# chalharu/rust-compression

Hardware: AMD Instinct MI355X
Metric: BZip2 level-9 encode MB/s (input bytes, HBM-resident in and out: the kernels' rate; value_end_to_end is host buffer to host buffer at the C ABI) (higher is better)
Workload: dtype u8/u32

## Files before the change

rust-compression_amd/csrc/bzgpu.h:

```cpp
#pragma once
#include <hip/hip_runtime.h>
#include <stdint.h>
#include <stddef.h>

namespace bzgpu {

typedef uint8_t u8;
typedef uint16_t u16;
typedef uint32_t u32;
typedef uint64_t u64;
typedef int64_t i64;

constexpr u32 kWave = 64;
constexpr u32 kMaxBlockLen = 900000;
constexpr u32 kSortTile = 8192;
constexpr u32 kSortThreads = 512;
constexpr u32 kTilesPerBlock = 110;
constexpr u32 kSlot = kTilesPerBlock * kSortTile;
constexpr u32 kMaxBins = 2048;
constexpr u32 kPerK = 8;
constexpr u32 kGSize = 50;
constexpr u32 kMaxSelectors = 18002;
constexpr u32 kMaxAlpha = 258;
constexpr u32 kRleTile = 4096;
// ... 248 lines not shown
    u32 *bin_base;
    u32 *count;
    u32 *count2;
    u32 *tile_nf;
    u8 *flags;
    u64 *newbits;
    int *tile_last_old;
    int *tile_last_new;
    u32 *nonfinal;
    unsigned long long *active;
    u32 *maxnf;
    u32 *per_k, *per_shift;
    u32 *lin_p, *lin_sig;
    u32 *bin_cursor;
    u32 *pb_gate;
    u32 *loc_stats;
    u8 *L;
    u32 *orig_ptr;
    u8 *ptext;
    const u8 *sym_code;
    const u8 *keyinfo;
    u32 *gh_tiles;
    u32 *gbase;
    u32 *tile_state;
    u32 *tickets;
    u32 *sort_err;
    u32 *epoch;
    u8 *per_aux;
    u32 per_keyshift;
    u32 per_wide;
    u32 per_links;
    u32 *fused_state;
    u32 *tile_state_all;
    u32 fused;
    size_t tile_state_bytes;
};
constexpr u32 kSortEpochs = 1024;

constexpr u32 kMtfStride = kSlot + 64;
struct MtfArgs {
    const BlockDesc *blocks;
    u32 nb;
    u32 tiles;
    const u8 *L;
    const u32 *inuse_bits;
    u8 *summ;
    u16 *summ_len;
    u8 *init_state;
    u8 *rank8;
    int *ztile_last;
    u32 *ztile_cnt;
    u32 *zstate;
    u32 *ztick;
    u32 fused_zle;
    u16 *mtf;
    u32 *mtf_freq;
    BlockOut *out;
};

constexpr u32 kLim = 17;
constexpr u32 kLmRow = 2 * kMaxAlpha + 4;
constexpr u32 kLmWords = 2 * kLim * kLmRow + 5 * kMaxAlpha + 64;
constexpr u32 kSelStride = kMaxSelectors + 14;
constexpr u32 kGboStride = kMaxSelectors + 2;
struct HuffArgs {
    const BlockDesc *blocks;
    u32 nb;
    const u16 *mtf;
    u32 mtf_stride;
    const u32 *mtf_freq;
    const u32 *inuse_bits;
    const u32 *crc;
    const u32 *orig_ptr;
    u8 *selector;
    u32 *code_len;
    u32 *group_bitoff;
    u32 *lm_scratch;
    u8 *glen;
    unsigned long long *pack;
    u32 *rfreq;
    u32 *hlm;
    u32 *pass_stats;
    u32 *stream;
    BlockOut *out;
    u32 *error_flag;
};

struct AsmBlock {
    u64 src_word;
    u64 bit_len;
    u64 dst_bit;
};
struct PackBlock {
    u64 src_word, dst_word, nwords;
};

constexpr int BZ_DEC_E_DATA = -1;
struct DecCand {
    u64 bitpos;
    u32 type;
    u32 pad;
};
struct DecBlockInfo {
    u64 end_bit;
    u32 status;
    u32 stored_crc;
// ... 139 lines not shown
```

rust-compression_amd/csrc/engine.hip:

```cpp
#include "engine_state.h"

#include <algorithm>
#include <chrono>
#include <cstdio>
#include <cstdlib>
#include <cstring>
#include <vector>


#define MAILCHK(st, ...)                                                             \
    do {                                                                             \
        const MailSeg mail_segs_[] = {__VA_ARGS__};                                  \
        if (mail_fetch((st), mail_segs_, (int)(sizeof(mail_segs_) / sizeof(mail_segs_[0]))) != 0) return BZ_E_UNEXPECTED; \
    } while (0)

static int span_begin(bz_gpu_engine *g, int stage, hipStream_t st = nullptr)
{
    bz_gpu_engine::Span s;
    s.stage = stage;
    s.st = st ? st : g->st;
    if (hipEventCreate(&s.a) != hipSuccess || hipEventCreate(&s.b) != hipSuccess) return -1;
    (void)hipEventRecord(s.a, s.st);
    g->spans.push_back(s);
    return (int)g->spans.size() - 1;
// ... 26 lines not shown
static int ensure_workspace(bz_gpu_engine *g, size_t need_blocks)
{
    if (need_blocks > g->max_blocks) need_blocks = g->max_blocks;
    if (need_blocks < 8) need_blocks = 8;
    if (g->ws_blocks >= need_blocks) return BZ_OK;
    size_t nb = need_blocks + need_blocks / 4;
    if (nb > g->max_blocks) nb = g->max_blocks;
    int rc = BZ_OK;
    g->ws_blocks = 0;
#define ENS(buf, bytes)                         \
    do {                                        \
        rc = g->buf.ensure((size_t)(bytes));    \
        if (rc != BZ_OK) return rc;             \
    } while (0)
    ENS(lblocks, nb * sizeof(BlockDesc));
    ENS(lcrc, nb * 4);
    ENS(SA, nb * (size_t)kSlot * 4);
    ENS(R, nb * (size_t)kSlot * 4);
    ENS(KA, nb * (size_t)kSlot * 4);
    ENS(VA, nb * (size_t)kSlot * 4);
    ENS(KB, nb * (size_t)kSlot * 4);
    ENS(VB, nb * (size_t)kSlot * 4);
    ENS(tile_hist, nb * (size_t)kTilesPerBlock * kMaxBins * 4);
    ENS(count, nb * 4);
    ENS(bin_base, nb * (size_t)kMaxBins * 4);
    ENS(sym_code, nb * (size_t)256);
    ENS(count2, nb * 4);
    ENS(tile_nf, nb * (size_t)kTilesPerBlock * 4);
    ENS(keyinfo, nb * (size_t)4);
    ENS(flags, nb * (size_t)kSlot);
    ENS(newbits, nb * (size_t)kSlot / 8 + 256);
    ENS(tlo, nb * (size_t)kTilesPerBlock * 4);
    ENS(tln, nb * (size_t)kTilesPerBlock * 4);
    ENS(nonfinal, nb * 4);
    ENS(active, 64 * 8 + 64 * 4);
    ENS(per_k, nb * 4);
    ENS(per_shift, nb * 4);
    ENS(lin_p, nb * (size_t)4 * kPerK);
    ENS(lin_sig, nb * (size_t)4 * kPerK);
    ENS(bin_cursor, nb * (size_t)1024 * 4);
    ENS(pb_gate, nb * (size_t)4 + 1024);
    if (hipMemsetAsync(g->pb_gate.p, 0, g->pb_gate.cap, g->st) != hipSuccess) return BZ_E_UNEXPECTED;
    ENS(L, nb * (size_t)kSlot + 64);
    ENS(orig_ptr, nb * 4);
    ENS(inuse_bits, nb * 32);
    ENS(summ, nb * (size_t)kMaxMtfChunks * 256);
    ENS(summ_len, nb * (size_t)kMaxMtfChunks * 2);
    ENS(init_state, nb * (size_t)kMaxMtfChunks * 256);
    ENS(rank8, nb * (size_t)kSlot + 64);
    ENS(ztile_last, nb * (size_t)kTilesPerBlock * 4);
    ENS(ztile_cnt, nb * (size_t)kTilesPerBlock * 4);
    ENS(zstate, nb * (size_t)kTilesPerBlock * 16);
    ENS(ztick, 64);
    ENS(mtf, nb * (size_t)kMtfStride * 2);
    ENS(mtf_freq, nb * (size_t)kMaxAlpha * 4);
    ENS(bout, nb * sizeof(BlockOut));
    ENS(selector, nb * (size_t)kSelStride);
    ENS(code_len, nb * (size_t)6 * kMaxAlpha * 4);
    ENS(group_bitoff, nb * (size_t)kGboStride * 4);
    ENS(lm_scratch, nb * (size_t)6 * kLmWords * 4);
    ENS(hglen, nb * (size_t)6 * (kMaxAlpha + 6));
    ENS(hpack, nb * (size_t)kMaxAlpha * 8);
    ENS(hrfreq, nb * (size_t)6 * kMaxAlpha * 4);
    ENS(hlm, nb * 4);
    ENS(hpass, nb * (size_t)32 * 4);
    ENS(stream, nb * (size_t)kStreamWords * 4);
    ENS(error_flag, 4);
    ENS(packlist, nb * sizeof(PackBlock));
    if (fused_wanted()) {
        ENS(gh_tiles, nb * (size_t)kTilesPerBlock * 3 * kMaxBins * 4);
        ENS(gbase, nb * (size_t)3 * kMaxBins * 4);
        ENS(tile_state, nb * (size_t)kTilesPerBlock * kMaxBins * 4);
        ENS(tickets, (size_t)kSortEpochs * 8 * 4 + 64);
        if (hipMemsetAsync(g->tile_state.p, 0, g->tile_state.cap, g->st) != hipSuccess ||
            hipMemsetAsync(g->tickets.p, 0, g->tickets.cap, g->st) != hipSuccess)
            return BZ_E_UNEXPECTED;
        g->sort_epoch = 0;
    }
#undef ENS
    g->ws_blocks = nb;
    return BZ_OK;
}

extern "C" int bz_device_count(void)
{
    int n = 0;
    if (hipGetDeviceCount(&n) != hipSuccess) return 0;
    return n;
}

extern "C" size_t bz_encode_bound(size_t n)
{
    return n + n / 2 + (n / 700000 + 2) * 24576 + 64;
}

extern "C" int bz_gpu_engine_create(bz_gpu_engine **out, int device, size_t max_blocks_in_flight)
{
    if (!out) return BZ_E_PARAM;
    *out = nullptr;
    int ndev = 0;
    if (hipGetDeviceCount(&ndev) != hipSuccess || ndev <= 0) return BZ_E_NOGPU;
    if (device < 0 || device >= ndev) return BZ_E_PARAM;
    HIPCHK(hipSetDevice(device));
    bz_gpu_engine *g = new bz_gpu_engine();
    g->device = device;
    g->max_blocks = max_blocks_in_flight ? max_blocks_in_flight : 64;
    g->verify = bzgpu::env_verify();
    HIPCHK(hipStreamCreateWithFlags(&g->st, hipStreamNonBlocking));
    HIPCHK(hipStreamCreateWithFlags(&g->st2, hipStreamNonBlocking));
    HIPCHK(hipHostMalloc((void **)&g->h_active, 64, hipHostMallocDefault));

    u32 tab[256], xp16[256], xp2[48];
    for (u32 i = 0; i < 256; ++i) {
        u32 v = i << 24;
        for (int k = 0; k < 8; ++k) v = (v & 0x80000000u) ? ((v << 1) ^ kCrcPoly) : (v << 1);
        tab[i] = v;
    }
    xp2[0] = 0x100u;
    for (int k = 1; k < 48; ++k) xp2[k] = gf_mulmod(xp2[k - 1], xp2[k - 1]);
    xp16[0] = 1u;
    for (int k = 1; k < 256; ++k) xp16[k] = gf_mulmod(xp16[k - 1], xp2[4]);
    int rc;
    if ((rc = g->crc_tab.ensure(sizeof(tab))) || (rc = g->xp16.ensure(sizeof(xp16))) ||
        (rc = g->xp2.ensure(sizeof(xp2)))) {
        delete g;
        return rc;
    }
    HIPCHK(hipMemcpy(g->crc_tab.p, tab, sizeof(tab), hipMemcpyHostToDevice));
    HIPCHK(hipMemcpy(g->xp16.p, xp16, sizeof(xp16), hipMemcpyHostToDevice));
    HIPCHK(hipMemcpy(g->xp2.p, xp2, sizeof(xp2), hipMemcpyHostToDevice));
    *out = g;
    return BZ_OK;
}

extern "C" int bz_gpu_engine_reserve(bz_gpu_engine *g, size_t blocks)
{
    if (!g) return BZ_E_PARAM;
    HIPCHK(hipSetDevice(g->device));
    return ensure_workspace(g, blocks);
}

extern "C" void bz_gpu_engine_destroy(bz_gpu_engine *g)
{
    if (!g) return;
    (void)hipSetDevice(g->device);
    (void)hipStreamSynchronize(g->st);
    (void)hipStreamSynchronize(g->st2);
    DevBuf *all[] = {&g->dec_in, &g->oneshot_out, &g->cut_step_t0, &g->cut_step_nt, &g->cut_step_w0, &g->cut_tab, &g->cut_comp,
                     &g->crc_tab, &g->xp16, &g->xp2, &g->tile_last, &g->carry_in, &g->tile_crc, &g->tile_count,
                     &g->tile_off, &g->sub_off, &g->sub_rs, &g->scal, &g->scan_part, &g->rle, &g->blocks_all, &g->crc_all, &g->lblocks, &g->lcrc, &g->SA,
                     &g->R, &g->KA, &g->VA, &g->KB, &g->VB, &g->tile_hist, &g->count, &g->flags, &g->tlo, &g->tln,
                     &g->nonfinal, &g->active, &g->per_k, &g->per_shift, &g->lin_p, &g->lin_sig, &g->bin_cursor, &g->pb_gate, &g->newbits, &g->bin_base, &g->sym_code, &g->keyinfo, &g->count2, &g->tile_nf, &g->L, &g->orig_ptr, &g->inuse_bits,
                     &g->summ, &g->summ_len, &g->init_state, &g->rank8, &g->ztile_last, &g->ztile_cnt, &g->mtf,
                     &g->mtf_freq, &g->bout, &g->selector, &g->code_len, &g->group_bitoff, &g->lm_scratch, &g->hglen, &g->hpack, &g->hrfreq, &g->hlm, &g->hpass,
                     &g->stream, &g->error_flag, &g->packlist, &g->packed, &g->gathered, &g->asmlist, &g->gh_tiles, &g->gbase, &g->tile_state,
                     &g->tickets, &g->vstream, &g->vout, &g->vseg, &g->vmis};
    for (DevBuf *b : all) b->release();
    dec_workspace_free(g->dec);
    df_workspace_free(g->df);
    if (g->h_active) (void)hipHostFree(g->h_active);
    if (g->st) (void)hipStreamDestroy(g->st);
    if (g->ev_aux) (void)hipEventDestroy(g->ev_aux);
    if (g->st2) (void)hipStreamDestroy(g->st2);
    delete g;
}

static RleBuffers rle_buffers(bz_gpu_engine *g)
{
    RleBuffers rb;
    rb.tile_last = g->tile_last.as<i64>();
    rb.carry_in = g->carry_in.as<i64>();
    rb.tile_crc = g->tile_crc.as<u32>();
    rb.tile_count = g->tile_count.as<u32>();
    rb.tile_off = g->tile_off.as<u64>();
    rb.sub_off = g->sub_off.as<u16>();
    rb.sub_rs = g->sub_rs.as<i64>();
    rb.total = g->scal.as<u64>();
    rb.cut_result = g->scal.as<u64>() + 2;
    rb.scan_part = g->scan_part.as<u64>();
    return rb;
}

extern "C" int bz_gpu_partition_slab_begin(bz_gpu_engine *g, int level, const void *d_in, size_t n,
                                           uint64_t tile0, uint64_t tile1, int64_t *slab_last_start)
{
    if (!g || level < 1 || level > 9) return BZ_E_PARAM;
    if (n && ((uintptr_t)d_in & 15u)) return BZ_E_PARAM;
    HIPCHK(hipSetDevice(g->device));
    const u64 ntiles = (n + kRleTile - 1) / kRleTile;
    if (tile1 > ntiles) tile1 = ntiles;
    if (tile0 > tile1) tile0 = tile1;
    g->level = level;
    g->d_in = (const u8 *)d_in;
    g->n_in = n;
    g->slab_t0 = tile0;
    g->slab_t1 = tile1;
    g->h_blocks.clear();
    g->h_crc.clear();
    for (double &t : g->t_stage) t = 0;
    for (u64 &s : g->bwt_stats) s = 0;
    for (u64 &s : g->round_active) s = 0;
    if (slab_last_start) *slab_last_start = -1;
    if (ntiles == 0) return BZ_OK;
    int rc;
    if ((rc = g->tile_last.ensure(ntiles * 8)) || (rc = g->carry_in.ensure(ntiles * 8)) ||
        (rc = g->tile_crc.ensure(ntiles * 4)) || (rc = g->tile_count.ensure(ntiles * 4)) ||
// ... 368 lines not shown
    x.tile_last_old = g->tlo.as<int>() + t;
    x.tile_last_new = g->tln.as<int>() + t;
    x.nonfinal = g->nonfinal.as<u32>() + o;
    x.active = g->active.as<unsigned long long>();
    x.maxnf = reinterpret_cast<u32 *>(g->active.as<unsigned long long>() + 64);
    x.per_k = g->per_k.as<u32>() + o;
    x.per_shift = g->per_shift.as<u32>() + o;
    x.lin_p = g->lin_p.as<u32>() + (size_t)o * kPerK;
    x.lin_sig = g->lin_sig.as<u32>() + (size_t)o * kPerK;
    x.bin_cursor = g->bin_cursor.as<u32>() + (size_t)o * 1024;
    x.pb_gate = g->pb_gate.as<u32>() + o;
    x.loc_stats = g->pb_gate.as<u32>() + g->ws_blocks;
    x.L = g->L.as<u8>() + s;
    x.orig_ptr = g->orig_ptr.as<u32>() + o;
    x.ptext = g->rank8.as<u8>() + s;
    x.sym_code = g->sym_code.as<u8>() + (size_t)o * 256;
    x.keyinfo = g->keyinfo.as<u8>() + (size_t)o * 4;
    x.gh_tiles = g->gh_tiles.as<u32>() + t * 3 * kMaxBins;
    x.gbase = g->gbase.as<u32>() + (size_t)o * 3 * kMaxBins;
    x.tile_state = g->tile_state.as<u32>() + t * kMaxBins;
    x.tickets = g->tickets.as<u32>();
    x.sort_err = g->tickets.p ? g->tickets.as<u32>() + (size_t)kSortEpochs * 8 : nullptr;
    x.epoch = &g->sort_epoch;
    x.fused_state = g->fused_state;
    x.tile_state_all = g->tile_state.as<u32>();
    x.tile_state_bytes = g->tile_state.cap;
    x.fused = fused_wanted() ? 1u : 0u;
    static const u32 want_links = (getenv("BZ_LINK_ROUND") && atoi(getenv("BZ_LINK_ROUND")) == 0) ? 0u : 1u;
    x.per_links = want_links;
    x.per_keyshift = 0;
    x.per_wide = 0;
    x.per_aux = reinterpret_cast<u8 *>(g->mtf.as<u16>() + (size_t)o * kMtfStride);
    return x;
}

static MtfArgs make_mtf_args(bz_gpu_engine *g, u32 nb, u32 o, u32 total_nb)
{
    MtfArgs ma;
    const size_t s = (size_t)o * kSlot, t = (size_t)o * kTilesPerBlock, c = (size_t)o * kMaxMtfChunks;
    ma.blocks = g->lblocks.as<BlockDesc>() + o;
    ma.nb = nb;
    ma.tiles = kTilesPerBlock;
    ma.L = g->L.as<u8>() + s;
    ma.inuse_bits = g->inuse_bits.as<u32>() + (size_t)o * 8;
    ma.summ = g->summ.as<u8>() + c * 256;
    ma.summ_len = g->summ_len.as<u16>() + c;
    ma.init_state = g->init_state.as<u8>() + c * 256;
    ma.rank8 = g->rank8.as<u8>() + s;
    ma.ztile_last = g->ztile_last.as<int>() + t;
    ma.ztile_cnt = g->ztile_cnt.as<u32>() + t;
    ma.zstate = g->zstate.as<u32>() + t * 4;
    ma.ztick = g->ztick.as<u32>();
    static const bool want_fused_zle = !(getenv("BZ_FUSED_ZLE") && atoi(getenv("BZ_FUSED_ZLE")) == 0);
    ma.fused_zle = (want_fused_zle && !g->zle_fused_broken && o == 0 && nb == total_nb) ? 1u : 0u;
    ma.mtf = g->mtf.as<u16>() + (size_t)o * kMtfStride;
    ma.mtf_freq = g->mtf_freq.as<u32>() + (size_t)o * kMaxAlpha;
    ma.out = g->bout.as<BlockOut>() + o;
    return ma;
}

static HuffArgs make_huff_args(bz_gpu_engine *g, u32 nb, u32 o)
{
    HuffArgs ha;
    ha.blocks = g->lblocks.as<BlockDesc>() + o;
    ha.nb = nb;
    ha.mtf = g->mtf.as<u16>() + (size_t)o * kMtfStride;
    ha.mtf_stride = kMtfStride;
    ha.mtf_freq = g->mtf_freq.as<u32>() + (size_t)o * kMaxAlpha;
    ha.inuse_bits = g->inuse_bits.as<u32>() + (size_t)o * 8;
    ha.crc = g->lcrc.as<u32>() + o;
    ha.orig_ptr = g->orig_ptr.as<u32>() + o;
    ha.selector = g->selector.as<u8>() + (size_t)o * kSelStride;
    ha.code_len = g->code_len.as<u32>() + (size_t)o * 6 * kMaxAlpha;
    ha.group_bitoff = g->group_bitoff.as<u32>() + (size_t)o * kGboStride;
    ha.lm_scratch = g->lm_scratch.as<u32>() + (size_t)o * 6 * kLmWords;
    ha.glen = g->hglen.as<u8>() + (size_t)o * 6 * (kMaxAlpha + 6);
    ha.pack = g->hpack.as<unsigned long long>() + (size_t)o * kMaxAlpha;
    ha.rfreq = g->hrfreq.as<u32>() + (size_t)o * 6 * kMaxAlpha;
    ha.hlm = g->hlm.as<u32>() + o;
    ha.pass_stats = g->debug_figures ? g->hpass.as<u32>() + (size_t)o * 32 : nullptr;
    ha.stream = g->stream.as<u32>() + (size_t)o * kStreamWords;
    ha.out = g->bout.as<BlockOut>() + o;
    ha.error_flag = g->error_flag.as<u32>();
    return ha;
}

__global__ void k_test_bump(u32 *p, u32 n) { *p = (*p + 1u) % n; }
__global__ void k_test_swap(u8 *L, u32 n)
{
    for (u32 i = n / 2; i + 1 < n; ++i)
        if (L[i] != L[i + 1]) {
            const u8 t = L[i];
            L[i] = L[i + 1];
            L[i + 1] = t;
            return;
        }
}

static int sort_batch(bz_gpu_engine *g, const BwtArgs &ba, u32 *inuse_bits, u32 max_n, u64 total_n, u64 *sorted,
                      KernelProf *prof, u64 *round_active)
{
    launch_block_symbols(g->st, ba, inuse_bits, const_cast<u8 *>(ba.sym_code), const_cast<u8 *>(ba.keyinfo));
    std::vector<u8> ki((size_t)ba.nb * 4);
    {
        const MailSeg sg = {ki.data(), ba.keyinfo, ki.size()};
        if (mail_fetch(g->st, &sg, 1) != 0) return -1;
    }
// ... 874 lines not shown
```

rust-compression_amd/csrc/engine_state.h:

```cpp
#pragma once
#include "../../include/bz2_mi355x.h"
#include "bzgpu.h"

#include <cstdio>
#include <vector>

using namespace bzgpu;

struct DecWorkspace;
void dec_workspace_free(DecWorkspace *w);
int dec_decode_for_verify(struct bz_gpu_engine *g, const uint8_t *d_in, uint64_t n, uint8_t *d_out, uint64_t cap,
                          uint64_t *produced, int *verdict);
struct bz_gpu_engine *dec_cache_take(int device, int prefer = 0);
void dec_cache_put(int device, struct bz_gpu_engine *g);
void dec_release_cached();
struct DfWorkspace;
void df_workspace_free(DfWorkspace *w);

#define HIPCHK(x)                                                                                     \
    do {                                                                                              \
        hipError_t e_ = (x);                                                                          \
        if (e_ != hipSuccess) {                                                                       \
            fprintf(stderr, "bz2_mi355x: HIP error %s at %s:%d\n", hipGetErrorString(e_), __FILE__,   \
                    __LINE__);                                                                        \
            return BZ_E_UNEXPECTED;                                                                   \
        }                                                                                             \
    } while (0)

struct DevBuf {
    void *p = nullptr;
    size_t cap = 0;
    int ensure(size_t bytes)
    {
        if (bytes <= cap) return BZ_OK;
        if (p) (void)hipFree(p);
        p = nullptr;
        cap = 0;
        size_t want = bytes + bytes / 8 + 256;
        if (hipMalloc(&p, want) != hipSuccess) {
            if (hipMalloc(&p, bytes) != hipSuccess) return BZ_E_NOMEM;
            want = bytes;
        }
        cap = want;
        return BZ_OK;
    }
    void release()
    {
        if (p) (void)hipFree(p);
        p = nullptr;
        cap = 0;
    }
    template <class T> T *as() const { return reinterpret_cast<T *>(p); }
};

struct bz_gpu_engine {
    int device = 0;
    hipStream_t st = nullptr;
    hipStream_t st2 = nullptr;
    size_t max_blocks = 0;

    DevBuf crc_tab, xp16, xp2;
    DevBuf tile_last, carry_in, tile_crc, tile_count, tile_off, sub_off, sub_rs, scal, scan_part, rle, blocks_all, crc_all;
    DevBuf cut_step_t0, cut_step_nt, cut_step_w0, cut_tab, cut_comp;
    CutPlan cut_plan = {};
    bool cut_ready = false;
    u64 h_halo_total = 0;
    u64 cut_stats[2] = {0, 0};
    std::vector<BlockDesc> h_blocks;
    std::vector<u32> h_crc;
    const u8 *d_in = nullptr;
    u64 n_in = 0;
    u64 slab_t0 = 0, slab_t1 = 0;
    int level = 9;
    DevBuf lblocks, lcrc, SA, R, KA, VA, KB, VB, tile_hist, count, flags, tlo, tln, nonfinal, active, per_k,
        per_shift, lin_p, lin_sig, bin_cursor, pb_gate, bin_base, newbits, sym_code, keyinfo, count2, tile_nf, L, orig_ptr, inuse_bits, summ, summ_len, init_state, rank8, ztile_last, ztile_cnt, zstate, ztick, mtf,
        mtf_freq, bout, selector, code_len, group_bitoff, lm_scratch, hglen, hpack, hrfreq, hlm, hpass, stream, error_flag, packlist, gh_tiles, gbase,
        tile_state, tickets;
    u32 sort_epoch = 0;
    bool zle_fused_broken = false;
    u32 fused_state[2] = {0, 0};
    hipEvent_t ev_aux = nullptr;
    size_t ws_blocks = 0;
    DevBuf packed, gathered, asmlist;
    unsigned long long *h_active = nullptr;
    std::vector<BlockOut> h_out;
    std::vector<u32> h_out_nblock;
    std::vector<u32> h_out_pass;
    double t_stage[6] = {0, 0, 0, 0, 0, 0};
    KernelProf prof;
    double shard_ms[8] = {0, 0, 0, 0, 0, 0, 0, 0};
    u64 bwt_stats[4] = {0, 0, 0, 0};
    u64 round_active[64] = {};

    struct Span {
        int stage;
        hipStream_t st;
        hipEvent_t a, b;
    };
    std::vector<Span> spans;
    bool verify = false;
    bool debug_figures = false;
    u64 verify_stats[4] = {0, 0, 0, 0};
    DevBuf vstream, vout, vseg, vmis;
    DecWorkspace *dec = nullptr;
    DevBuf dec_in, oneshot_out;
    DfWorkspace *df = nullptr;
};
```

rust-compression_amd/csrc/k_mtf.hip:

```cpp
#include "bzgpu.h"
#include <cstdlib>

namespace bzgpu {

constexpr u32 kChunkWGs = (kMaxMtfChunks + 255) / 256;
constexpr u32 kMtfSmallAlpha = 96;

__device__ __forceinline__ u32 popc8(const u32 *b)
{
    u32 c = 0;
#pragma unroll
    for (int i = 0; i < 8; ++i) c += __popc(b[i]);
    return c;
}

__global__ __launch_bounds__(256) void k_mtf_summaries(MtfArgs a)
{
    __shared__ u32 s_seen[8 * 256];
    const u32 lb = blockIdx.y;
    const u32 n = a.blocks[lb].n;
    const u32 chunk = blockIdx.x * 256u + threadIdx.x;
    const u32 beg = chunk * kMtfChunk;
    if (beg >= n) return;
    const u32 end = (beg + kMtfChunk < n) ? beg + kMtfChunk : n;
// ... 85 lines not shown
    u32 len = a.summ_len[rep0 + c0];
    reinterpret_cast<u32 *>(s_cur)[l] = act ? reinterpret_cast<const u32 *>(a.summ + (rep0 + c0) * 256u)[l] : 0u;
    __syncthreads();
    u32 c1 = c0 + kMtfGroup;
    if (c1 > nchunks - 1u) c1 = nchunks - 1u;
    u32 m_next = c0 + 1u < c1 ? (u32)a.summ_len[rep0 + c0 + 1u] : 0u;
    u32 w_next = (c0 + 1u < c1 && act) ? reinterpret_cast<const u32 *>(a.summ + (rep0 + c0 + 1u) * 256u)[l] : 0u;
    for (u32 c = c0 + 1u; c < c1; ++c) {
        const u32 m = m_next, w = w_next;
        if (c + 1u < c1) {
            m_next = a.summ_len[rep0 + c + 1u];
            w_next = act ? reinterpret_cast<const u32 *>(a.summ + (rep0 + c + 1u) * 256u)[l] : 0u;
        }
        len = mtf_apply_report(s_cur, len, m, w, s_new, s_mark, l);
        if (act) reinterpret_cast<u32 *>(a.summ + (rep0 + c) * 256u)[l] = reinterpret_cast<u32 *>(s_cur)[l];
        if (l == 0) a.summ_len[rep0 + c] = (u16)len;
    }
}

__global__ __launch_bounds__(64) void k_mtf_group_starts(MtfArgs a)
{
    __shared__ u8 s_state[256], s_new[256], s_mark[256];
    const u32 lb = blockIdx.x, l = threadIdx.x;
    const u32 n = a.blocks[lb].n;
    const u32 nchunks = (n + kMtfChunk - 1) / kMtfChunk;
    const u32 *bits = a.inuse_bits + lb * 8;
    {
        u32 before = 0;
        for (u32 q = 0; q < (l * 4u) / 32u; ++q) before += __popc(bits[q]);
        const u32 wd = bits[(l * 4u) >> 5];
        const u32 sh = (l * 4u) & 31u;
        before += __popc(wd & ((1u << sh) - 1u));
        reinterpret_cast<u32 *>(s_state)[l] = 0;
        __syncthreads();
        u32 pos = before;
        for (u32 k = 0; k < 4; ++k)
            if ((wd >> (sh + k)) & 1u) s_state[pos++] = (u8)(l * 4u + k);
    }
    __syncthreads();
    const u32 alpha = popc8(bits);
    const size_t rep0 = (size_t)lb * kMaxMtfChunks;
    const bool act = l * 4u < alpha;
    for (u32 c0 = 0; c0 < nchunks; c0 += kMtfGroup) {
        if (act) reinterpret_cast<u32 *>(a.init_state + (rep0 + c0) * 256u)[l] = reinterpret_cast<u32 *>(s_state)[l];
        if (c0 + 2u > nchunks) break;
        u32 e = c0 + kMtfGroup - 1u;
        if (e > nchunks - 2u) e = nchunks - 2u;
        const u32 m = a.summ_len[rep0 + e];
        const u32 w = act ? reinterpret_cast<const u32 *>(a.summ + (rep0 + e) * 256u)[l] : 0u;
        (void)mtf_apply_report(s_state, alpha, m, w, s_new, s_mark, l);
    }
}

__global__ __launch_bounds__(256) void k_mtf_chunk_starts(MtfArgs a)
{
    __shared__ u8 s_state[4][256], s_new[4][256], s_mark[4][256];
    const u32 lb = blockIdx.y, l = threadIdx.x & 63u, wv = threadIdx.x >> 6;
    const u32 n = a.blocks[lb].n;
    const u32 nchunks = (n + kMtfChunk - 1) / kMtfChunk;
    const u32 c0 = blockIdx.x * kMtfGroup;
    if (c0 + 1u >= nchunks) return;
    const u32 alpha = popc8(a.inuse_bits + lb * 8);
    const size_t rep0 = (size_t)lb * kMaxMtfChunks;
    const bool act = l * 4u < alpha;
    const u32 g32 = act ? reinterpret_cast<const u32 *>(a.init_state + (rep0 + c0) * 256u)[l] : 0u;
    for (u32 k = 0; k < kMtfGroup / 4u; ++k) {
        const u32 c = c0 + 1u + k * 4u + wv;
        const bool live = c < nchunks && c < c0 + kMtfGroup;
        reinterpret_cast<u32 *>(s_state[wv])[l] = g32;
        const u32 m = live ? (u32)a.summ_len[rep0 + c - 1u] : 0u;
        const u32 w = (live && act) ? reinterpret_cast<const u32 *>(a.summ + (rep0 + c - 1u) * 256u)[l] : 0u;
        (void)mtf_apply_report(s_state[wv], alpha, m, w, s_new[wv], s_mark[wv], l);
        if (live && act) reinterpret_cast<u32 *>(a.init_state + (rep0 + c) * 256u)[l] = reinterpret_cast<u32 *>(s_state[wv])[l];
    }
}


constexpr u32 kMtfSmallPairs = kMtfSmallAlpha / 2;
constexpr u32 kMtfSubBlocks = 16;
typedef short short2_t __attribute__((ext_vector_type(2)));
__device__ __forceinline__ short2_t as_short2(u32 v)
{
    short2_t r;
    __builtin_memcpy(&r, &v, 4);
    return r;
}
template <u32 PAIRS, u32 LANES, u32 ALPHA_LO, u32 SUB = 1>
__global__ __launch_bounds__(LANES) void k_mtf_ranks_small(MtfArgs a)
{
    constexpr u32 CL = LANES / SUB;
    __shared__ u32 s_last[PAIRS * CL];
    __shared__ u8 s_code[256];
    const u32 lb = blockIdx.y;
    const u32 n = a.blocks[lb].n;
    const u32 chunk0 = blockIdx.x * CL;
    const u32 sub = threadIdx.x % SUB;
    if (chunk0 * kMtfChunk >= n) return;
    const u32 *bits = a.inuse_bits + lb * 8;
    const u32 alpha = popc8(bits);
    if (alpha > 2u * PAIRS || alpha <= ALPHA_LO) return;
    for (u32 v = threadIdx.x; v < 256u; v += LANES) {
        u32 before = 0;
        for (u32 q = 0; q < (v >> 5); ++q) before += __popc(bits[q]);
        before += __popc(bits[v >> 5] & ((1u << (v & 31u)) - 1u));
        s_code[v] = (u8)before;
    }
    __syncthreads();
    const u32 chunk = chunk0 + threadIdx.x / SUB;
    const u32 beg = chunk * kMtfChunk;
    if (beg >= n) return;
    const u32 end = (beg + kMtfChunk < n) ? beg + kMtfChunk : n;
    const u32 npairs = (alpha + 1u) >> 1;
    u32 *my = s_last + threadIdx.x / SUB;
    constexpr u32 kPB = 32;
    static_assert(PAIRS % (2u * kPB) == 0 || PAIRS <= kMtfSmallPairs, "the compare loop takes the table two blocks at a time");
    const u32 npairs16 = ((npairs + 2u * kPB - 1u) / (2u * kPB) * (2u * kPB)) < PAIRS ? ((npairs + 2u * kPB - 1u) / (2u * kPB) * (2u * kPB)) : PAIRS;
    for (u32 q = sub; q < (SUB > 1 ? PAIRS : npairs16); q += SUB) my[q * CL] = 0x80008000u;
    if (SUB > 1) {
        __builtin_amdgcn_fence(__ATOMIC_ACQ_REL, "workgroup");
        __builtin_amdgcn_wave_barrier();
    }
    if (sub == 0) {
        const u8 *st = a.init_state + ((size_t)lb * kMaxMtfChunks + chunk) * 256u;
        for (u32 q = 0; q < alpha; ++q) {
            const u32 c = s_code[st[q]];
            const u32 t = (u32)(0xFFFFu - q) & 0xFFFFu;
            u32 wd = my[(c >> 1) * CL];
            wd = (c & 1u) ? ((wd & 0x0000FFFFu) | (t << 16)) : ((wd & 0xFFFF0000u) | t);
            my[(c >> 1) * CL] = wd;
        }
    }
    if (SUB > 1) {
        __builtin_amdgcn_fence(__ATOMIC_ACQ_REL, "workgroup");
        __builtin_amdgcn_wave_barrier();
    }
    const u8 *L = a.L + (size_t)lb * kSlot;
    u8 *R8 = a.rank8 + (size_t)lb * kSlot;
    for (u32 v4 = 0; v4 < kMtfChunk / 64u; ++v4) {
        if (beg + v4 * 64u >= end) break;
        uint4 q4[4];
#pragma unroll
        for (u32 u = 0; u < 4; ++u) {
            const u32 pl = beg + v4 * 64u + u * 16u;
            q4[u] = (pl < end) ? *reinterpret_cast<const uint4 *>(L + pl) : make_uint4(0, 0, 0, 0);
        }
#pragma unroll
      for (u32 u = 0; u < 4; ++u) {
        const u32 v = v4 * 4u + u;
        const u32 p0 = beg + v * 16u;
        if (p0 >= end) break;
        const u32 wv[4] = {q4[u].x, q4[u].y, q4[u].z, q4[u].w};
        u32 ov[4] = {0, 0, 0, 0};
#pragma unroll
        for (u32 k = 0; k < 16; ++k) {
            u32 rank = 0;
            if (p0 + k < end) {
                const u32 c = s_code[(wv[k >> 2] >> ((k & 3) * 8)) & 0xFFu];
                const u32 wc = my[(c >> 1) * CL];
                const u32 lsu = (c & 1u) ? (wc >> 16) : (wc & 0xFFFFu);
                const short2_t ls2 = as_short2(lsu | (lsu << 16));
                short2_t acc = {0, 0};
              if (SUB == 1 && PAIRS > kMtfSmallPairs) {
                u32 ra[kPB], rb[kPB];
#pragma unroll
                for (u32 e = 0; e < kPB; ++e) ra[e] = my[e * CL];
                for (u32 q = 0; q < npairs16; q += 2u * kPB) {
#pragma unroll
                    for (u32 e = 0; e < kPB; ++e) rb[e] = my[(q + kPB + e) * CL];
#pragma unroll
                    for (u32 e = 0; e < kPB; ++e) acc -= __builtin_elementwise_sub_sat(ls2, as_short2(ra[e])) >> (short2_t){15, 15};
                    const u32 qn = (q + 2u * kPB < npairs16) ? q + 2u * kPB : 0u;
#pragma unroll
                    for (u32 e = 0; e < kPB; ++e) ra[e] = my[(qn + e) * CL];
#pragma unroll
                    for (u32 e = 0; e < kPB; ++e) acc -= __builtin_elementwise_sub_sat(ls2, as_short2(rb[e])) >> (short2_t){15, 15};
                }
              } else if (SUB > 1) {
                constexpr u32 PER = PAIRS / SUB;
                u32 ra[PER];
#pragma unroll
                for (u32 e = 0; e < PER; ++e) ra[e] = my[(sub * PER + e) * CL];
#pragma unroll
                for (u32 e = 0; e < PER; ++e) acc -= __builtin_elementwise_sub_sat(ls2, as_short2(ra[e])) >> (short2_t){15, 15};
              } else
                for (u32 q = 0; q < npairs; ++q) {
                    const short2_t wd = as_short2(my[q * CL]);
                    const short2_t neg = __builtin_elementwise_sub_sat(ls2, wd) >> (short2_t){15, 15};
                    acc -= neg;
                }
                rank = (u32)(int)acc.x + (u32)(int)acc.y;
                if (SUB > 1) {
#pragma unroll
                    for (u32 d = 1; d < SUB; d <<= 1) rank += (u32)__shfl_xor((int)rank, (int)d, 64);
                }
                const u32 t = (v * 16u + k) & 0xFFFFu;
                if (sub == 0) my[(c >> 1) * CL] = (c & 1u) ? ((wc & 0x0000FFFFu) | (t << 16)) : ((wc & 0xFFFF0000u) | t);
            }
            ov[k >> 2] |= rank << ((k & 3) * 8);
        }
        if (sub == 0) *reinterpret_cast<uint4 *>(R8 + p0) = make_uint4(ov[0], ov[1], ov[2], ov[3]);
      }
    }
}

struct ZSeg {
    u8 r[16];
    u32 valid;
    u32 p0;
    int next_nonzero;
};

__device__ __forceinline__ void zload(const u8 *__restrict__ R8, u32 n, u32 tile, ZSeg &s)
{
    s.p0 = tile * kSortTile + threadIdx.x * 16u;
    s.valid = s.p0 < n ? ((n - s.p0) < 16u ? (n - s.p0) : 16u) : 0u;
    if (s.valid) {
        const uint4 q = *reinterpret_cast<const uint4 *>(R8 + s.p0);
        const u32 wv[4] = {q.x, q.y, q.z, q.w};
#pragma unroll
        for (int k = 0; k < 16; ++k) s.r[k] = (u8)(wv[k >> 2] >> ((k & 3) * 8));
        const u32 nx = s.p0 + s.valid;
        s.next_nonzero = (nx >= n) ? 1 : (R8[nx] != 0);
    } else {
        s.next_nonzero = 1;
    }
}

__device__ __forceinline__ int block_excl_max_int(int v, int *sh )
{
    const u32 l = lane_id(), w = threadIdx.x >> 6;
    const int inc = wave_incl_max32(v);
    if (l == 63) sh[w] = inc;
    __syncthreads();
    int carry = -1;
    for (u32 k = 0; k < w; ++k) carry = sh[k] > carry ? sh[k] : carry;
    const int prev = __shfl_up(inc, 1, 64);
    const int ex = (l == 0) ? -1 : prev;
    __syncthreads();
    return ex > carry ? ex : carry;
}

__device__ __forceinline__ u32 block_excl_sum1024(u32 v, u32 *sh , u32 &total)
{
    const u32 l = lane_id(), w = threadIdx.x >> 6;
    const u32 inc = wave_incl_sum(v);
    if (l == 63) sh[w] = inc;
    __syncthreads();
    u32 carry = 0, tot = 0;
    for (u32 k = 0; k < kSortThreads / 64; ++k) {
        if (k < w) carry += sh[k];
        tot += sh[k];
    }
    total = tot;
    __syncthreads();
    return carry + inc - v;
}

__global__ __launch_bounds__(kSortThreads) void k_zle_last(MtfArgs a)
{
    __shared__ int s_last;
    const u32 lb = blockIdx.y, tile = blockIdx.x;
    const u32 n = a.blocks[lb].n;
    if (tile * kSortTile >= n) return;
    if (threadIdx.x == 0) s_last = -1;
    __syncthreads();
    ZSeg s;
    zload(a.rank8 + (size_t)lb * kSlot, n, tile, s);
    int last = -1;
#pragma unroll
    for (u32 k = 0; k < 16; ++k)
        if (k < s.valid && s.r[k]) last = (int)(s.p0 + k);
#pragma unroll
    for (u32 dd = 32; dd >= 1; dd >>= 1) {
        const int o = __shfl_xor(last, dd, 64);
        last = o > last ? o : last;
    }
    if (lane_id() == 0 && last >= 0) atomicMax(&s_last, last);
    __syncthreads();
    if (threadIdx.x == 0) a.ztile_last[lb * kTilesPerBlock + tile] = s_last;
}

__device__ __forceinline__ u32 run_digits(u32 z) { return 31u - (u32)__clz(z + 1u); }

template <bool WRITE>
__global__ __launch_bounds__(kSortThreads) void k_zle_emit(MtfArgs a)
{
    __shared__ int s_mi[16];
    __shared__ u32 s_su[16];
    __shared__ u32 s_freq[kMaxAlpha + 2];
    __shared__ int s_carry;
    __shared__ u32 s_base;
    __shared__ u16 s_out[WRITE ? kSortTile + 64 : 1];
    const u32 lb = blockIdx.y, tile = blockIdx.x;
    const u32 n = a.blocks[lb].n;
    if (tile * kSortTile >= n) return;
    if (threadIdx.x == 0) {
        int c = -1;
        for (int t = (int)tile - 1; t >= 0 && c < 0; --t) c = a.ztile_last[lb * kTilesPerBlock + t];
        s_carry = c;
        if (WRITE) {
            u32 b = 0;
            for (u32 t = 0; t < tile; ++t) b += a.ztile_cnt[lb * kTilesPerBlock + t];
            s_base = b;
        }
    }
    if (WRITE)
        for (u32 i = threadIdx.x; i < kMaxAlpha + 2; i += kSortThreads) s_freq[i] = 0;
    __syncthreads();
    ZSeg s;
    zload(a.rank8 + (size_t)lb * kSlot, n, tile, s);
    int last = -1;
#pragma unroll
    for (u32 k = 0; k < 16; ++k)
        if (k < s.valid && s.r[k]) last = (int)(s.p0 + k);
    int lnz = block_excl_max_int(last, s_mi);
    lnz = lnz > s_carry ? lnz : s_carry;
    u32 cnt = 0;
    {
        int ln = lnz;
#pragma unroll
        for (u32 k = 0; k < 16; ++k) {
            if (k < s.valid) {
                const u32 p = s.p0 + k;
                if (s.r[k]) {
                    ln = (int)p;
                    cnt += 1;
                } else {
                    const bool run_end = (k + 1 < s.valid) ? (s.r[(k + 1) & 15] != 0) : (s.next_nonzero != 0);
                    if (run_end) cnt += run_digits((u32)((int)p - ln));
                }
            }
        }
    }
    u32 total;
    u32 off = block_excl_sum1024(cnt, s_su, total);
// ... 176 lines not shown
    hot0 = wave_sum(hot0);
    hot1 = wave_sum(hot1);
    hot2 = wave_sum(hot2);
    hot3 = wave_sum(hot3);
    if ((threadIdx.x & 63u) == 0) {
        if (hot0) atomicAdd(&s_freq[0], hot0);
        if (hot1) atomicAdd(&s_freq[1], hot1);
        if (hot2) atomicAdd(&s_freq[2], hot2);
        if (hot3) atomicAdd(&s_freq[3], hot3);
    }
    if (threadIdx.x == 0) {
        u32 base = 0;
        if (tile) {
            u32 spins = 0;
            for (u32 p = tile; p > 0;) {
                --p;
                const u32 *src = a.zstate + ((size_t)lb * kTilesPerBlock + p) * 4u;
                uint4 v = ld_sc1_x4(src);
                while ((v.y & kLbFlagMask) == 0u) {
                    if (lb_give_up(spins, a.ztick + 8, kLbSpinMax >> 3)) {
                        atomicExch(a.ztick + 8, 1u);
                        v = make_uint4(0u, kLbIncl, 0u, 0u);
                        break;
                    }
                    __builtin_amdgcn_s_sleep(2);
                    v = ld_sc1_x4(src);
                }
                base += v.y & kLbValMask;
                if ((v.y & kLbFlagMask) == kLbIncl) break;
            }
            st_sc1_x4(mystate, make_uint4(w_last, kLbIncl | ((base + total) & kLbValMask), 0u, 0u));
        }
        s_base = base;
    }
    __syncthreads();
    {
        u16 *dst = a.mtf + (size_t)lb * kMtfStride + s_base;
        for (u32 i = threadIdx.x; i < total; i += kSortThreads) dst[i] = s_out[i];
    }
    const bool last_tile = (tile + 1) * kSortTile >= n;
    if (last_tile && threadIdx.x == 0) {
        const u32 alpha_in = popc8(a.inuse_bits + lb * 8);
        const u32 eob = alpha_in + 1u;
        a.mtf[(size_t)lb * kMtfStride + s_base + total] = (u16)eob;
        atomicAdd(&s_freq[eob], 1u);
        a.out[lb].mtf_count = s_base + total + 1u;
        a.out[lb].in_use_count = alpha_in;
    }
    __syncthreads();
    for (u32 i = threadIdx.x; i < kMaxAlpha; i += kSortThreads)
        if (s_freq[i]) atomicAdd(&a.mtf_freq[(size_t)lb * kMaxAlpha + i], s_freq[i]);
}

void launch_mtf(hipStream_t st, const MtfArgs &a)
{
    (void)hipMemsetAsync(a.mtf_freq, 0, (size_t)a.nb * kMaxAlpha * sizeof(u32), st);
    hipLaunchKernelGGL(k_mtf_summaries, dim3(kChunkWGs, a.nb), dim3(256), 0, st, a);
    hipLaunchKernelGGL(k_mtf_merge_groups, dim3(kMtfGroups, a.nb), dim3(64), 0, st, a);
    hipLaunchKernelGGL(k_mtf_group_starts, dim3(a.nb), dim3(64), 0, st, a);
    hipLaunchKernelGGL(k_mtf_chunk_starts, dim3(kMtfGroups, a.nb), dim3(256), 0, st, a);
    if (a.nb <= kMtfSubBlocks) {
        hipLaunchKernelGGL((k_mtf_ranks_small<kMtfSmallPairs, 256, 0, 8>), dim3((kMaxMtfChunks + 31) / 32, a.nb), dim3(256), 0, st, a);
        hipLaunchKernelGGL((k_mtf_ranks_small<128, 128, kMtfSmallAlpha, 8>), dim3((kMaxMtfChunks + 15) / 16, a.nb), dim3(128), 0, st, a);
    } else {
        hipLaunchKernelGGL((k_mtf_ranks_small<kMtfSmallPairs, 256, 0>), dim3(kChunkWGs, a.nb), dim3(256), 0, st, a);
        hipLaunchKernelGGL((k_mtf_ranks_small<128, 128, kMtfSmallAlpha>), dim3((kMaxMtfChunks + 127) / 128, a.nb), dim3(128), 0, st, a);
    }
    if (a.fused_zle) {
        (void)hipMemsetAsync(a.zstate, 0, (size_t)a.nb * kTilesPerBlock * 16, st);
        (void)hipMemsetAsync(a.ztick, 0, 64, st);
        hipLaunchKernelGGL(k_zle_fused, dim3(a.tiles, xcd_grid_y(a.nb)), dim3(kSortThreads), 0, st, a);
        return;
    }
    const dim3 grid(a.tiles, a.nb);
    hipLaunchKernelGGL(k_zle_last, grid, dim3(kSortThreads), 0, st, a);
    hipLaunchKernelGGL((k_zle_emit<false>), grid, dim3(kSortThreads), 0, st, a);
    hipLaunchKernelGGL((k_zle_emit<true>), grid, dim3(kSortThreads), 0, st, a);
}

}
```

Before: 13680.

## Stream zero-run encoding via per-chunk records and drop chunk-start kernel

Removes the k_mtf_chunk_starts kernel. The ranks kernel now rebuilds each chunk's initial MTF state from the previous chunk's summary plus its group's start state. The ranks kernel also records the first and last nonzero rank and the run-length symbol count for each chunk. A single-workgroup-per-block scan kernel then turns those records into output offsets and carries. A per-wave streaming kernel emits the zero-run and MTF symbols directly, replacing the fused decoupled-lookback ZLE path and the two-pass last/emit path. This cuts a kernel launch and the inter-tile serialization, at the cost of more per-thread work in the ranks kernel and a new zrec buffer.

```diff
diff --git a/rust-compression_amd/csrc/bzgpu.h b/rust-compression_amd/csrc/bzgpu.h
--- a/rust-compression_amd/csrc/bzgpu.h
+++ b/rust-compression_amd/csrc/bzgpu.h
@@ -324,6 +324,8 @@
     u32 *ztile_cnt;
     u32 *zstate;
     u32 *ztick;
+    uint4 *zrec;
+    u32 zle_stream;
     u32 fused_zle;
     u16 *mtf;
     u32 *mtf_freq;
diff --git a/rust-compression_amd/csrc/engine.hip b/rust-compression_amd/csrc/engine.hip
--- a/rust-compression_amd/csrc/engine.hip
+++ b/rust-compression_amd/csrc/engine.hip
@@ -102,6 +102,7 @@
     ENS(ztile_cnt, nb * (size_t)kTilesPerBlock * 4);
     ENS(zstate, nb * (size_t)kTilesPerBlock * 16);
     ENS(ztick, 64);
+    ENS(zrec, nb * (size_t)kMaxMtfChunks * 16);
     ENS(mtf, nb * (size_t)kMtfStride * 2);
     ENS(mtf_freq, nb * (size_t)kMaxAlpha * 4);
     ENS(bout, nb * sizeof(BlockOut));
@@ -201,7 +202,7 @@
                      &g->tile_off, &g->sub_off, &g->sub_rs, &g->scal, &g->scan_part, &g->rle, &g->blocks_all, &g->crc_all, &g->lblocks, &g->lcrc, &g->SA,
                      &g->R, &g->KA, &g->VA, &g->KB, &g->VB, &g->tile_hist, &g->count, &g->flags, &g->tlo, &g->tln,
                      &g->nonfinal, &g->active, &g->per_k, &g->per_shift, &g->lin_p, &g->lin_sig, &g->bin_cursor, &g->pb_gate, &g->newbits, &g->bin_base, &g->sym_code, &g->keyinfo, &g->count2, &g->tile_nf, &g->L, &g->orig_ptr, &g->inuse_bits,
-                     &g->summ, &g->summ_len, &g->init_state, &g->rank8, &g->ztile_last, &g->ztile_cnt, &g->mtf,
+                     &g->summ, &g->summ_len, &g->init_state, &g->rank8, &g->ztile_last, &g->ztile_cnt, &g->zrec, &g->mtf,
                      &g->mtf_freq, &g->bout, &g->selector, &g->code_len, &g->group_bitoff, &g->lm_scratch, &g->hglen, &g->hpack, &g->hrfreq, &g->hlm, &g->hpass,
                      &g->stream, &g->error_flag, &g->packlist, &g->packed, &g->gathered, &g->asmlist, &g->gh_tiles, &g->gbase, &g->tile_state,
                      &g->tickets, &g->vstream, &g->vout, &g->vseg, &g->vmis};
@@ -676,7 +677,11 @@
     ma.zstate = g->zstate.as<u32>() + t * 4;
     ma.ztick = g->ztick.as<u32>();
     static const bool want_fused_zle = !(getenv("BZ_FUSED_ZLE") && atoi(getenv("BZ_FUSED_ZLE")) == 0);
-    ma.fused_zle = (want_fused_zle && !g->zle_fused_broken && o == 0 && nb == total_nb) ? 1u : 0u;
+    static const bool want_zle_stream = !(getenv("BZ_ZLE_STREAM") && atoi(getenv("BZ_ZLE_STREAM")) == 0) &&
+                                        getenv("BZ_FUSED_ZLE_FAILTEST") == nullptr;
+    ma.zrec = g->zrec.as<uint4>() + c;
+    ma.zle_stream = (want_fused_zle && want_zle_stream && !g->zle_fused_broken) ? 1u : 0u;
+    ma.fused_zle = (!ma.zle_stream && want_fused_zle && !g->zle_fused_broken && o == 0 && nb == total_nb) ? 1u : 0u;
     ma.mtf = g->mtf.as<u16>() + (size_t)o * kMtfStride;
     ma.mtf_freq = g->mtf_freq.as<u32>() + (size_t)o * kMaxAlpha;
     ma.out = g->bout.as<BlockOut>() + o;
diff --git a/rust-compression_amd/csrc/engine_state.h b/rust-compression_amd/csrc/engine_state.h
--- a/rust-compression_amd/csrc/engine_state.h
+++ b/rust-compression_amd/csrc/engine_state.h
@@ -73,7 +73,7 @@
     u64 slab_t0 = 0, slab_t1 = 0;
     int level = 9;
     DevBuf lblocks, lcrc, SA, R, KA, VA, KB, VB, tile_hist, count, flags, tlo, tln, nonfinal, active, per_k,
-        per_shift, lin_p, lin_sig, bin_cursor, pb_gate, bin_base, newbits, sym_code, keyinfo, count2, tile_nf, L, orig_ptr, inuse_bits, summ, summ_len, init_state, rank8, ztile_last, ztile_cnt, zstate, ztick, mtf,
+        per_shift, lin_p, lin_sig, bin_cursor, pb_gate, bin_base, newbits, sym_code, keyinfo, count2, tile_nf, L, orig_ptr, inuse_bits, summ, summ_len, init_state, rank8, ztile_last, ztile_cnt, zstate, ztick, zrec, mtf,
         mtf_freq, bout, selector, code_len, group_bitoff, lm_scratch, hglen, hpack, hrfreq, hlm, hpass, stream, error_flag, packlist, gh_tiles, gbase,
         tile_state, tickets;
     u32 sort_epoch = 0;
diff --git a/rust-compression_amd/csrc/k_mtf.hip b/rust-compression_amd/csrc/k_mtf.hip
--- a/rust-compression_amd/csrc/k_mtf.hip
+++ b/rust-compression_amd/csrc/k_mtf.hip
@@ -161,29 +161,8 @@
     }
 }
 
-__global__ __launch_bounds__(256) void k_mtf_chunk_starts(MtfArgs a)
-{
-    __shared__ u8 s_state[4][256], s_new[4][256], s_mark[4][256];
-    const u32 lb = blockIdx.y, l = threadIdx.x & 63u, wv = threadIdx.x >> 6;
-    const u32 n = a.blocks[lb].n;
-    const u32 nchunks = (n + kMtfChunk - 1) / kMtfChunk;
-    const u32 c0 = blockIdx.x * kMtfGroup;
-    if (c0 + 1u >= nchunks) return;
-    const u32 alpha = popc8(a.inuse_bits + lb * 8);
-    const size_t rep0 = (size_t)lb * kMaxMtfChunks;
-    const bool act = l * 4u < alpha;
-    const u32 g32 = act ? reinterpret_cast<const u32 *>(a.init_state + (rep0 + c0) * 256u)[l] : 0u;
-    for (u32 k = 0; k < kMtfGroup / 4u; ++k) {
-        const u32 c = c0 + 1u + k * 4u + wv;
-        const bool live = c < nchunks && c < c0 + kMtfGroup;
-        reinterpret_cast<u32 *>(s_state[wv])[l] = g32;
-        const u32 m = live ? (u32)a.summ_len[rep0 + c - 1u] : 0u;
-        const u32 w = (live && act) ? reinterpret_cast<const u32 *>(a.summ + (rep0 + c - 1u) * 256u)[l] : 0u;
-        (void)mtf_apply_report(s_state[wv], alpha, m, w, s_new[wv], s_mark[wv], l);
-        if (live && act) reinterpret_cast<u32 *>(a.init_state + (rep0 + c) * 256u)[l] = reinterpret_cast<u32 *>(s_state[wv])[l];
-    }
-}
-
+__device__ __forceinline__ u32 run_digits(u32 z) { return 31u - (u32)__clz(z + 1u); }
+constexpr u32 kZNone = 0xFFFFFFFFu;
 
 constexpr u32 kMtfSmallPairs = kMtfSmallAlpha / 2;
 constexpr u32 kMtfSubBlocks = 16;
@@ -230,13 +209,42 @@
         __builtin_amdgcn_wave_barrier();
     }
     if (sub == 0) {
-        const u8 *st = a.init_state + ((size_t)lb * kMaxMtfChunks + chunk) * 256u;
-        for (u32 q = 0; q < alpha; ++q) {
-            const u32 c = s_code[st[q]];
-            const u32 t = (u32)(0xFFFFu - q) & 0xFFFFu;
-            u32 wd = my[(c >> 1) * CL];
-            wd = (c & 1u) ? ((wd & 0x0000FFFFu) | (t << 16)) : ((wd & 0xFFFF0000u) | t);
-            my[(c >> 1) * CL] = wd;
+        const size_t rep0 = (size_t)lb * kMaxMtfChunks;
+        const u32 g0 = chunk / kMtfGroup * kMtfGroup;
+        u32 q = 0;
+        if (chunk != g0) {
+            const uint4 *rp = reinterpret_cast<const uint4 *>(a.summ + (rep0 + chunk - 1u) * 256u);
+            const u32 m = a.summ_len[rep0 + chunk - 1u];
+            for (u32 q0 = 0; q0 < m; q0 += 16u) {
+                const uint4 v = rp[q0 >> 4];
+                const u32 wv[4] = {v.x, v.y, v.z, v.w};
+#pragma unroll
+                for (u32 k = 0; k < 16; ++k) {
+                    if (q0 + k >= m) break;
+                    const u32 c = s_code[(wv[k >> 2] >> ((k & 3) * 8)) & 0xFFu];
+                    const u32 t = (u32)(0xFFFFu - (q0 + k)) & 0xFFFFu;
+                    u32 wd = my[(c >> 1) * CL];
+                    wd = (c & 1u) ? ((wd & 0x0000FFFFu) | (t << 16)) : ((wd & 0xFFFF0000u) | t);
+                    my[(c >> 1) * CL] = wd;
+                }
+            }
+            q = m;
+        }
+        const uint4 *st = reinterpret_cast<const uint4 *>(a.init_state + (rep0 + g0) * 256u);
+        for (u32 j0 = 0; j0 < alpha && q < alpha; j0 += 16u) {
+            const uint4 v = st[j0 >> 4];
+            const u32 wv[4] = {v.x, v.y, v.z, v.w};
+#pragma unroll
+            for (u32 k = 0; k < 16; ++k) {
+                if (j0 + k >= alpha) break;
+                const u32 c = s_code[(wv[k >> 2] >> ((k & 3) * 8)) & 0xFFu];
+                u32 wd = my[(c >> 1) * CL];
+                if (((c & 1u) ? (wd >> 16) : (wd & 0xFFFFu)) != 0x8000u) continue;
+                const u32 t = (u32)(0xFFFFu - q) & 0xFFFFu;
+                wd = (c & 1u) ? ((wd & 0x0000FFFFu) | (t << 16)) : ((wd & 0xFFFF0000u) | t);
+                my[(c >> 1) * CL] = wd;
+                ++q;
+            }
         }
     }
     if (SUB > 1) {
@@ -245,6 +253,8 @@
     }
     const u8 *L = a.L + (size_t)lb * kSlot;
     u8 *R8 = a.rank8 + (size_t)lb * kSlot;
+    int fnz = -1, lnz = -1;
+    u32 inner = 0;
     for (u32 v4 = 0; v4 < kMtfChunk / 64u; ++v4) {
         if (beg + v4 * 64u >= end) break;
         uint4 q4[4];
@@ -304,12 +314,19 @@
                 }
                 const u32 t = (v * 16u + k) & 0xFFFFu;
                 if (sub == 0) my[(c >> 1) * CL] = (c & 1u) ? ((wc & 0x0000FFFFu) | (t << 16)) : ((wc & 0xFFFF0000u) | t);
+                if (rank) {
+                    inner += 1u + (fnz >= 0 ? run_digits(t - 1u - (u32)lnz) : 0u);
+                    fnz = fnz >= 0 ? fnz : (int)t;
+                    lnz = (int)t;
+                }
             }
             ov[k >> 2] |= rank << ((k & 3) * 8);
         }
         if (sub == 0) *reinterpret_cast<uint4 *>(R8 + p0) = make_uint4(ov[0], ov[1], ov[2], ov[3]);
       }
     }
+    if (a.zle_stream && sub == 0)
+        a.zrec[(size_t)lb * kMaxMtfChunks + chunk] = make_uint4(fnz >= 0 ? beg + (u32)fnz : kZNone, lnz >= 0 ? beg + (u32)lnz : kZNone, inner, 0u);
 }
 
 struct ZSeg {
@@ -388,8 +405,6 @@
     __syncthreads();
     if (threadIdx.x == 0) a.ztile_last[lb * kTilesPerBlock + tile] = s_last;
 }
-
-__device__ __forceinline__ u32 run_digits(u32 z) { return 31u - (u32)__clz(z + 1u); }
 
 template <bool WRITE>
 __global__ __launch_bounds__(kSortThreads) void k_zle_emit(MtfArgs a)
@@ -672,13 +687,163 @@
         if (s_freq[i]) atomicAdd(&a.mtf_freq[(size_t)lb * kMaxAlpha + i], s_freq[i]);
 }
 
+constexpr u32 kZScanPer = (kMaxMtfChunks + kSortThreads - 1) / kSortThreads;
+__global__ __launch_bounds__(kSortThreads) void k_zle_scan(MtfArgs a)
+{
+    __shared__ int s_mi[16];
+    __shared__ u32 s_su[16];
+    const u32 lb = blockIdx.x;
+    const u32 n = a.blocks[lb].n;
+    if (n == 0) return;
+    const u32 nchunks = (n + kMtfChunk - 1) / kMtfChunk;
+    uint4 *rec = a.zrec + (size_t)lb * kMaxMtfChunks;
+    const u32 c0 = threadIdx.x * kZScanPer;
+    int f[kZScanPer], l[kZScanPer];
+    u32 cnt[kZScanPer];
+    int tl = -1;
+#pragma unroll
+    for (u32 j = 0; j < kZScanPer; ++j) {
+        const uint4 r = (c0 + j < nchunks) ? rec[c0 + j] : make_uint4(kZNone, kZNone, 0u, 0u);
+        f[j] = (int)r.x;
+        l[j] = (int)r.y;
+        cnt[j] = r.z;
+        tl = l[j] > tl ? l[j] : tl;
+    }
+    const int f_next = (c0 + kZScanPer < nchunks) ? (int)rec[c0 + kZScanPer].x : -1;
+    int carry = block_excl_max_int(tl, s_mi);
+    int before[kZScanPer];
+    u32 sum = 0;
+#pragma unroll
+    for (u32 j = 0; j < kZScanPer; ++j) {
+        before[j] = carry;
+        if (c0 + j >= nchunks) continue;
+        const u32 b = (c0 + j) * kMtfChunk, e = (b + kMtfChunk < n) ? b + kMtfChunk : n;
+        if (f[j] > (int)b) cnt[j] += run_digits((u32)(f[j] - 1 - carry));
+        const int fn = (j + 1 < kZScanPer) ? f[j + 1] : f_next;
+        if (l[j] != (int)e - 1 && (e == n || fn == (int)e))
+            cnt[j] += run_digits((u32)((int)e - 1 - (l[j] >= 0 ? l[j] : carry)));
+        carry = l[j] >= 0 ? l[j] : carry;
+        sum += cnt[j];
+    }
+    u32 total;
+    u32 off = block_excl_sum1024(sum, s_su, total);
+#pragma unroll
+    for (u32 j = 0; j < kZScanPer; ++j)
+        if (c0 + j < nchunks) {
+            rec[c0 + j] = make_uint4((u32)before[j], off, 0u, 0u);
+            off += cnt[j];
+        }
+    if (threadIdx.x == 0) {
+        const u32 alpha_in = popc8(a.inuse_bits + lb * 8);
+        const u32 eob = alpha_in + 1u;
+        a.mtf[(size_t)lb * kMtfStride + total] = (u16)eob;
+        atomicAdd(&a.mtf_freq[(size_t)lb * kMaxAlpha + eob], 1u);
+        a.out[lb].mtf_count = total + 1u;
+        a.out[lb].in_use_count = alpha_in;
+    }
+}
+
+constexpr u32 kZWaveOut = 2 * kMtfChunk + 32;
+__global__ __launch_bounds__(kSortThreads) void k_zle_stream(MtfArgs a)
+{
+    __shared__ u32 s_freq[kMaxAlpha + 2];
+    __shared__ u16 s_out[kSortThreads / 64][kZWaveOut];
+    const u32 lb = blockIdx.y, tile = blockIdx.x;
+    const u32 n = a.blocks[lb].n;
+    if (tile * kSortTile >= n) return;
+    for (u32 i = threadIdx.x; i < kMaxAlpha + 2; i += kSortThreads) s_freq[i] = 0;
+    __syncthreads();
+    const u32 w = threadIdx.x >> 6, l = lane_id();
+    const u32 w0 = tile * kSortTile + w * 64u * 16u;
+    u32 hot0 = 0, hot1 = 0, hot2 = 0, hot3 = 0;
+    if (w0 < n) {
+        const uint4 rec = a.zrec[(size_t)lb * kMaxMtfChunks + w0 / kMtfChunk];
+        ZSeg s;
+        zload(a.rank8 + (size_t)lb * kSlot, n, tile, s);
+        int last = -1;
+#pragma unroll
+        for (u32 k = 0; k < 16; ++k)
+            if (k < s.valid && s.r[k]) last = (int)(s.p0 + k);
+        const int incl = wave_incl_max32(last);
+        const int prev = __shfl_up(incl, 1, 64);
+        int lnz = l ? prev : -1;
+        lnz = lnz > (int)rec.x ? lnz : (int)rec.x;
+        u32 cnt = 0;
+        {
+            int ln = lnz;
+#pragma unroll
+            for (u32 k = 0; k < 16; ++k) {
+                if (k < s.valid) {
+                    const u32 p = s.p0 + k;
+                    if (s.r[k]) {
+                        ln = (int)p;
+                        cnt += 1;
+                    } else {
+                        const bool run_end = (k + 1 < s.valid) ? (s.r[(k + 1) & 15] != 0) : (s.next_nonzero != 0);
+                        if (run_end) cnt += run_digits((u32)((int)p - ln));
+                    }
+                }
+            }
+        }
+        const u32 inc = wave_incl_sum(cnt);
+        const u32 wtot = __shfl(inc, 63, 64);
+        u16 *out = s_out[w] + (inc - cnt);
+        {
+            int ln = lnz;
+#pragma unroll
+            for (u32 k = 0; k < 16; ++k) {
+                if (k < s.valid) {
+                    const u32 p = s.p0 + k;
+                    if (s.r[k]) {
+                        ln = (int)p;
+                        const u32 sym = (u32)s.r[k] + 1u;
+                        *out++ = (u16)sym;
+                        if (sym == 2u) ++hot2;
+                        else if (sym == 3u) ++hot3;
+                        else atomicAdd(&s_freq[sym], 1u);
+                    } else {
+                        const bool run_end = (k + 1 < s.valid) ? (s.r[(k + 1) & 15] != 0) : (s.next_nonzero != 0);
+                        if (run_end) {
+                            u32 zc = (u32)((int)p - ln) + 1u;
+                            while (zc > 1u) {
+                                const u32 run = zc & 1u;
+                                *out++ = (u16)run;
+                                hot0 += run ^ 1u;
+                                hot1 += run;
+                                zc >>= 1;
+                            }
+                        }
+                    }
+                }
+            }
+        }
+        __builtin_amdgcn_fence(__ATOMIC_ACQ_REL, "workgroup");
+        __builtin_amdgcn_wave_barrier();
+        u16 *dst = a.mtf + (size_t)lb * kMtfStride + rec.y;
+        if (rec.y <= kSlot)
+            for (u32 i = l; i < wtot; i += 64u) dst[i] = s_out[w][i];
+    }
+    hot0 = wave_sum(hot0);
+    hot1 = wave_sum(hot1);
+    hot2 = wave_sum(hot2);
+    hot3 = wave_sum(hot3);
+    if (l == 0) {
+        if (hot0) atomicAdd(&s_freq[0], hot0);
+        if (hot1) atomicAdd(&s_freq[1], hot1);
+        if (hot2) atomicAdd(&s_freq[2], hot2);
+        if (hot3) atomicAdd(&s_freq[3], hot3);
+    }
+    __syncthreads();
+    for (u32 i = threadIdx.x; i < kMaxAlpha; i += kSortThreads)
+        if (s_freq[i]) atomicAdd(&a.mtf_freq[(size_t)lb * kMaxAlpha + i], s_freq[i]);
+}
+
 void launch_mtf(hipStream_t st, const MtfArgs &a)
 {
     (void)hipMemsetAsync(a.mtf_freq, 0, (size_t)a.nb * kMaxAlpha * sizeof(u32), st);
     hipLaunchKernelGGL(k_mtf_summaries, dim3(kChunkWGs, a.nb), dim3(256), 0, st, a);
     hipLaunchKernelGGL(k_mtf_merge_groups, dim3(kMtfGroups, a.nb), dim3(64), 0, st, a);
     hipLaunchKernelGGL(k_mtf_group_starts, dim3(a.nb), dim3(64), 0, st, a);
-    hipLaunchKernelGGL(k_mtf_chunk_starts, dim3(kMtfGroups, a.nb), dim3(256), 0, st, a);
     if (a.nb <= kMtfSubBlocks) {
         hipLaunchKernelGGL((k_mtf_ranks_small<kMtfSmallPairs, 256, 0, 8>), dim3((kMaxMtfChunks + 31) / 32, a.nb), dim3(256), 0, st, a);
         hipLaunchKernelGGL((k_mtf_ranks_small<128, 128, kMtfSmallAlpha, 8>), dim3((kMaxMtfChunks + 15) / 16, a.nb), dim3(128), 0, st, a);
@@ -686,6 +851,11 @@
         hipLaunchKernelGGL((k_mtf_ranks_small<kMtfSmallPairs, 256, 0>), dim3(kChunkWGs, a.nb), dim3(256), 0, st, a);
         hipLaunchKernelGGL((k_mtf_ranks_small<128, 128, kMtfSmallAlpha>), dim3((kMaxMtfChunks + 127) / 128, a.nb), dim3(128), 0, st, a);
     }
+    if (a.zle_stream) {
+        hipLaunchKernelGGL(k_zle_scan, dim3(a.nb), dim3(kSortThreads), 0, st, a);
+        hipLaunchKernelGGL(k_zle_stream, dim3(a.tiles, a.nb), dim3(kSortThreads), 0, st, a);
+        return;
+    }
     if (a.fused_zle) {
         (void)hipMemsetAsync(a.zstate, 0, (size_t)a.nb * kTilesPerBlock * 16, st);
         (void)hipMemsetAsync(a.ztick, 0, 64, st);
```

After: 13760 (median of 6 runs). About the same (+0.6%).
